# FifthEpoch/longcat-video-tta

Measured on AMD Instinct MI355X. Metric: denoised latent frames/sec (49x720p, 50-step CFG denoise), higher is better.
Workload: dtype bf16

## Files before the change

### longcat-video-tta_amd/csrc/attn_fwd_w64.hip

```cpp
#include "lcv_common.h"
#include <type_traits>

typedef __attribute__((address_space(3))) unsigned char lds_u8w;
#define AS3W __attribute__((address_space(3)))
#define SCHED_FENCE() __builtin_amdgcn_sched_barrier(0)

struct AttnFwdW64Params {
  const bf16_t* q;
  const bf16_t* k;
  const bf16_t* v;
  bf16_t* o;
  float* lse;
  int64_t Nq, Nk;
  int H;
  int64_t q_sb, q_sn, q_sh, k_sb, k_sn, k_sh, v_sb, v_sn, v_sh, o_sb, o_sn, o_sh;
  float scale;
  int gx, xcd_remap;
};

#define W64_RESCALE_THR 6.0f


__device__ __forceinline__ float w64_half_max(float v) {
  float a = v, b = v;
  asm volatile("s_nop 1\n\tv_permlane32_swap_b32 %0, %1\n\ts_nop 0" : "+v"(a), "+v"(b));
  return fmaxf(a, b);
}
__device__ __forceinline__ float w64_half_sum(float v) {
  float a = v, b = v;
  asm volatile("s_nop 1\n\tv_permlane32_swap_b32 %0, %1\n\ts_nop 0" : "+v"(a), "+v"(b));
  return a + b;
}
__device__ __forceinline__ float w_exp2(float x) { float y; asm volatile("v_exp_f32 %0, %1" : "=v"(y) : "v"(x)); return y; }
__device__ __forceinline__ float w_add(float a, float b) { float y; asm volatile("v_add_f32 %0, %1, %2" : "=v"(y) : "v"(a), "v"(b)); return y; }
__device__ __forceinline__ float w_max3(float a, float b, float c) { float y; asm volatile("v_max3_f32 %0, %1, %2, %3" : "=v"(y) : "v"(a), "v"(b), "v"(c)); return y; }
typedef __attribute__((ext_vector_type(2))) float f32x2w;
__device__ __forceinline__ f32x2w w_pk_add(f32x2w a, f32x2w b) { f32x2w y; asm volatile("v_pk_add_f32 %0, %1, %2" : "=v"(y) : "v"(a), "v"(b)); return y; }
__device__ __forceinline__ unsigned w_pack(float lo, float hi) { unsigned y; asm volatile("v_cvt_pk_bf16_f32 %0, %1, %2" : "=v"(y) : "v"(lo), "v"(hi)); return y; }

template <bool GUARD>
__device__ __forceinline__ void mfma_s(f32x16& c, const bf16x8& a, const bf16x8& b) {
  if constexpr (GUARD) asm volatile("s_nop 3\n\tv_mfma_f32_32x32x16_bf16 %0, %1, %2, %0" : "+v"(c) : "v"(a), "a"(b));
  else asm volatile("v_mfma_f32_32x32x16_bf16 %0, %1, %2, %0" : "+v"(c) : "v"(a), "a"(b));
}
template <bool GUARD>
__device__ __forceinline__ void mfma_s_first(f32x16& d, const f32x16& c, const bf16x8& a, const bf16x8& b) {
  if constexpr (GUARD) asm volatile("s_nop 3\n\tv_mfma_f32_32x32x16_bf16 %0, %2, %3, %1" : "=&v"(d) : "v"(c), "v"(a), "a"(b));
  else asm volatile("v_mfma_f32_32x32x16_bf16 %0, %2, %3, %1" : "=&v"(d) : "v"(c), "v"(a), "a"(b));
}
template <bool GUARD>
__device__ __forceinline__ void mfma_o(f32x16& c, const bf16x8& a, const bf16x8& b) {
  if constexpr (GUARD) asm volatile("s_nop 3\n\tv_mfma_f32_32x32x16_bf16 %0, %1, %2, %0" : "+a"(c) : "v"(a), "v"(b));
  else asm volatile("v_mfma_f32_32x32x16_bf16 %0, %1, %2, %0" : "+a"(c) : "v"(a), "v"(b));
}

#define SCW(S, nb, j) (S[(j) >> 4][nb][(j) & 15])

__global__ __launch_bounds__(256) void attn_fwd_w64_kernel(const AttnFwdW64Params p) {
  constexpr int TILE = 64 * 256;
  extern __shared__ __attribute__((aligned(16))) unsigned char smem[];
  lds_u8w* lds = (lds_u8w*)smem;
  constexpr int V_REGION = 2 * TILE;

  const int tid = threadIdx.x;
  const int lane = tid & 63;
  const int wave = __builtin_amdgcn_readfirstlane(tid >> 6);
  const int r = lane & 31, h = lane >> 5;
  int qb, head;
  int64_t b;
  if (p.xcd_remap) {
    const int id = blockIdx.x;
    const int xcd = id & 7, j = id >> 3;
    const int pair = (j / p.gx) * 8 + xcd;
    qb = j - (j / p.gx) * p.gx;
    head = pair % p.H;
    b = pair / p.H;
  } else {
    qb = blockIdx.x; head = blockIdx.y; b = blockIdx.z;
  }
  const int64_t q0 = (int64_t)qb * 256 + wave * 64;
  auto lane_now = []() -> int { return (int)__builtin_amdgcn_mbcnt_hi(~0u, __builtin_amdgcn_mbcnt_lo(~0u, 0u)); };
  const int nt = (int)((p.Nk + 63) / 64);
  const bool ragged = (p.Nk & 63) != 0;
  const char* kbase_u = lcv_uniform_ptr(p.k + b * p.k_sb + (int64_t)head * p.k_sh);
  const char* vbase_u = lcv_uniform_ptr(p.v + b * p.v_sb + (int64_t)head * p.v_sh);

  auto dma_row_of = [&](int ln, int i) { return 16 * wave + 4 * i + (ln >> 4); };
  auto dma_colb_of = [&](int ln, int i) {
    const int row = dma_row_of(ln, i);
    return 16 * ((ln & 15) ^ (((row & 3) << 2) | ((row >> 2) & 3)));
  };
  unsigned koff[4], voff[4];
#pragma unroll
  for (int i = 0; i < 4; ++i) {
    koff[i] = (unsigned)(dma_row_of(lane, i) * p.k_sn * 2 + dma_colb_of(lane, i));
    voff[i] = (unsigned)(dma_row_of(lane, i) * p.v_sn * 2 + dma_colb_of(lane, i));
  }
  auto last_off = [&](int i, int64_t sn) {
    const int ln = lane_now();
    int64_t row = (int64_t)(nt - 1) * 64 + dma_row_of(ln, i);
    if (row > p.Nk - 1) row = p.Nk - 1;
    return (unsigned)(row * sn * 2 + dma_colb_of(ln, i));
  };
  const unsigned lds_wave = (unsigned)(uintptr_t)lds + (unsigned)wave * 4096u;
  auto dma_one = [&](int which, int i, int dst_tile, int tile, bool known_full) __attribute__((always_inline)) {
    const int64_t sn = which ? p.v_sn : p.k_sn;
    const char* base = which ? vbase_u : kbase_u;
    unsigned off = which ? voff[i] : koff[i];
    if (!known_full && tile == nt - 1) off = last_off(i, sn);
    else base += (int64_t)tile * (128 * sn);
    asm volatile("s_mov_b32 m0, %2\n\ts_nop 0\n\tglobal_load_lds_dwordx4 %0, %1"
                 :: "v"(off), "s"(base), "s"(lds_wave + (unsigned)dst_tile + 1024u * i) : "memory", "m0");
  };
  auto dma_tile = [&](int which, int dst_tile, int tile) __attribute__((always_inline)) {
#pragma unroll
    for (int i = 0; i < 4; ++i) dma_one(which, i, dst_tile, tile, false);
  };
  constexpr int KOP = 0, VOP = 1;
  auto dma_wait_and_barrier = [&]() { asm volatile("s_waitcnt vmcnt(0)\n\ts_barrier" ::: "memory"); };

  int k_off[8];
  int v_off[2][4];
  auto set_read_offsets = [&](int ln, int slot) {
    const int rr = ln & 31, hh = ln >> 5;
    const int kfz = ((rr & 3) << 2) | ((rr >> 2) & 3);
#pragma unroll
    for (int ks = 0; ks < 8; ++ks) k_off[ks] = 256 * rr + 16 * ((2 * ks + hh) ^ kfz);
    const int q4 = (ln >> 2) & 3, p4 = ln & 3, g1 = (ln >> 4) & 1;
#pragma unroll
    for (int half = 0; half < 2; ++half)
#pragma unroll
      for (int d = 0; d < 4; ++d)
        v_off[half][d] = (int)(unsigned)(uintptr_t)lds + V_REGION + slot * TILE + 256 * (4 * hh + 8 * half + q4) + 8 * (p4 & 1) + 64 * (d ^ q4) +
                         16 * ((2 * g1 + (p4 >> 1)) ^ (hh + 2 * half));
  };
  set_read_offsets(lane, 2);
  auto read_k = [&](const lds_u8w* kb, int f) __attribute__((always_inline)) -> bf16x8 {
    return *reinterpret_cast<const AS3W bf16x8*>(kb + (f & 1) * 32 * 256 + k_off[f >> 1]);
  };
  auto read_v = [&](int g) __attribute__((always_inline)) -> bf16x8 {
    const s16x4 lo = __builtin_amdgcn_ds_read_tr16_b64_v4i16((AS3W s16x4*)(uintptr_t)(unsigned)(v_off[0][g & 3] + 4096 * (g >> 2)));
    const s16x4 hi = __builtin_amdgcn_ds_read_tr16_b64_v4i16((AS3W s16x4*)(uintptr_t)(unsigned)(v_off[1][g & 3] + 4096 * (g >> 2)));
    return __builtin_bit_cast(bf16x8, __builtin_shufflevector(lo, hi, 0, 1, 2, 3, 4, 5, 6, 7));
  };

  bf16x8 qf[2][8];
#pragma unroll
  for (int nb = 0; nb < 2; ++nb) {
    int64_t qrow = q0 + 32 * nb + r;
    if (qrow > p.Nq - 1) qrow = p.Nq - 1;
    const bf16_t* qp = p.q + b * p.q_sb + qrow * p.q_sn + (int64_t)head * p.q_sh + 8 * h;
#pragma unroll
    for (int ks = 0; ks < 8; ++ks) qf[nb][ks] = *reinterpret_cast<const bf16x8*>(qp + 16 * ks);
  }
#pragma unroll
  for (int nb = 0; nb < 2; ++nb)
#pragma unroll
    for (int ks = 0; ks < 8; ++ks) asm volatile("" : "+a"(qf[nb][ks]));

  f32x16 oacc[2][4];
#pragma unroll
  for (int nb = 0; nb < 2; ++nb)
#pragma unroll
    for (int d = 0; d < 4; ++d) {
#pragma unroll
      for (int e = 0; e < 16; ++e) oacc[nb][d][e] = 0.f;
      asm volatile("" : "+a"(oacc[nb][d]));
    }
  float m_run[2] = {0.f, 0.f}, l_run[2] = {0.f, 0.f};
  f32x16 minit[2];
#pragma unroll
  for (int nb = 0; nb < 2; ++nb)
#pragma unroll
    for (int e = 0; e < 16; ++e) minit[nb][e] = 0.f;
  f32x16 sa[2][2], sb[2][2];

  auto mask_last = [&](f32x16 (&s)[2][2]) __attribute__((always_inline)) {
    const int valid = (int)(p.Nk - (int64_t)(nt - 1) * 64);
    const int hh_ = lane_now() >> 5;
#pragma unroll
    for (int nb = 0; nb < 2; ++nb)
#pragma unroll
      for (int e = 0; e < 16; ++e) {
        const int key = (e & 3) + 8 * (e >> 2) + 4 * hh_;
        if (key >= valid) s[0][nb][e] = -INFINITY;
        if (key + 32 >= valid) s[1][nb][e] = -INFINITY;
      }
  };
  auto fence_o = [&]() __attribute__((always_inline)) {
    asm volatile("s_nop 15\n\ts_nop 15\n\ts_nop 15\n\ts_nop 15"
                 : "+a"(oacc[0][0]), "+a"(oacc[0][1]), "+a"(oacc[0][2]), "+a"(oacc[0][3]), "+a"(oacc[1][0]), "+a"(oacc[1][1]),
                   "+a"(oacc[1][2]), "+a"(oacc[1][3]));
  };
  auto fence_s = [&](f32x16 (&s)[2][2]) __attribute__((always_inline)) {
    asm volatile("s_nop 15\n\ts_nop 15\n\ts_nop 15\n\ts_nop 15" : "+v"(s[0][0]), "+v"(s[0][1]), "+v"(s[1][0]), "+v"(s[1][1]));
  };
  auto settle = [&](f32x16 (&s)[2][2], auto nb_c, float mx, bool first, bool need) __attribute__((always_inline)) {
    constexpr int nb = decltype(nb_c)::value;
    if (need || first) {
      fence_o();
      const float d = first ? mx : fmaxf(mx, 0.f);
      const float alpha = __builtin_amdgcn_exp2f(-d);
      m_run[nb] += d;
      l_run[nb] *= alpha;
#pragma unroll
      for (int dd = 0; dd < 4; ++dd)
#pragma unroll
        for (int e = 0; e < 16; ++e) oacc[nb][dd][e] *= alpha;
#pragma unroll
      for (int e = 0; e < 16; ++e) {
        s[0][nb][e] -= d;
        s[1][nb][e] -= d;
        asm volatile("v_mov_b32 %0, %1" : "+v"(minit[nb][e]) : "v"(-m_run[nb]));
      }
      fence_o();
    }
  };

#ifndef W64_PD
#define W64_PD 2
#endif
#ifndef W64_DMA_STRIDE
#define W64_DMA_STRIDE 1
#endif
  constexpr int PD = W64_PD, RING = PD + 1;
  bf16x8 kfr[RING], vfr[RING];
  int v_slot = 2;
  auto next_v_slot = [&]() __attribute__((always_inline)) -> int {
    v_slot = (v_slot == 2) ? 0 : v_slot + 1;
    return (v_slot == 0) ? -2 * TILE : TILE;
  };

  dma_tile(KOP, 0, 0);
  dma_tile(VOP, V_REGION, 0);
  dma_tile(KOP, TILE, 1);
  dma_tile(VOP, V_REGION + TILE, 1);
  dma_wait_and_barrier();
  {
#pragma unroll
    for (int kb_ = 0; kb_ < 2; ++kb_)
#pragma unroll
      for (int nb = 0; nb < 2; ++nb)
#pragma unroll
        for (int e = 0; e < 16; ++e) sa[kb_][nb][e] = 0.f;
#pragma unroll
    for (int f = 0; f < 16; ++f) {
      const bf16x8 a = read_k(lds, f);
      mfma_s<true>(sa[f & 1][0], a, qf[0][f >> 1]);
      mfma_s<true>(sa[f & 1][1], a, qf[1][f >> 1]);
    }
    fence_s(sa);
    auto first_settle = [&](auto nb_c) __attribute__((always_inline)) {
      constexpr int nb = decltype(nb_c)::value;
      float mx = sa[0][nb][0];
#pragma unroll
      for (int e = 1; e < 16; ++e) mx = fmaxf(mx, sa[0][nb][e]);
#pragma unroll
      for (int e = 0; e < 16; ++e) mx = fmaxf(mx, sa[1][nb][e]);
      settle(sa, nb_c, w64_half_max(mx), true, true);
    };
    first_settle(std::integral_constant<int, 0>{});
    first_settle(std::integral_constant<int, 1>{});
  }
  __syncthreads();
  dma_tile(KOP, 0, 2);
#pragma unroll
  for (int i = 0; i < PD; ++i) kfr[i] = read_k(lds + TILE, i);

  auto iteration = [&](const int t, auto par_c, auto steady_c, f32x16 (&c)[2][2], f32x16 (&n)[2][2]) __attribute__((always_inline)) {
    constexpr int PAR = decltype(par_c)::value;
    constexpr bool STEADY = decltype(steady_c)::value;
    const lds_u8w* kb = lds + (PAR ^ 1) * TILE;
    const lds_u8w* kb_next = lds + PAR * TILE;
    const bool has_k3 = STEADY || t + 3 < nt;
    const bool has_v2 = STEADY || t + 2 < nt;
    const int v_delta = next_v_slot();
    const int v_dst = V_REGION + ((v_slot == 0) ? 2 : v_slot - 1) * TILE;
    f32x2w psum[2];
    f32x2w ex[2][16];
    unsigned pw[2][16];
    SCHED_FENCE();
#pragma unroll
    for (int i = 0; i < 32; ++i) {
      const int f = i >> 1, nb = i & 1;
      if (nb == 0) {
        if (f + PD < 16) kfr[(f + PD) % RING] = read_k(kb, f + PD);
        if (f >= 16 - PD) vfr[f - (16 - PD)] = read_v(f - (16 - PD));
      }
      if (f < 2) {
        if (STEADY && i >= 1) mfma_s_first<false>(n[f & 1][nb], minit[nb], kfr[f % RING], qf[nb][0]);
        else mfma_s_first<true>(n[f & 1][nb], minit[nb], kfr[f % RING], qf[nb][0]);
      } else {
        if (STEADY) mfma_s<false>(n[f & 1][nb], kfr[f % RING], qf[nb][f >> 1]);
        else mfma_s<true>(n[f & 1][nb], kfr[f % RING], qf[nb][f >> 1]);
      }
      SCHED_FENCE();
      if (i >= 10 && i < 18) asm volatile("v_add_u32 %0, %1, %0" : "+v"(v_off[(i - 10) >> 2][(i - 10) & 3]) : "s"(v_delta));
      const int e_lo = (3 * i + 1) / 2, e_hi = (3 * (i + 1) + 1) / 2;
      const int a_lo = i ? (3 * (i - 1) + 1) / 2 : 0, a_hi = i ? e_lo : 0;
#pragma unroll
      for (int u = 0; u < 2; ++u) {
        const int x = e_lo + u;
        if (x < e_hi) ex[x & 1][x >> 2][(x >> 1) & 1] = w_exp2(SCW(c, x & 1, x >> 1));
      }
#pragma unroll
      for (int u = 0; u < 2; ++u) {
        const int x = a_lo + u;
        if (x < a_hi) {
          const int b_ = x & 1, j = x >> 1;
          if (j & 1) {
            pw[b_][j >> 1] = w_pack(ex[b_][j >> 1][0], ex[b_][j >> 1][1]);
            if (j == 3) psum[b_] = w_pk_add(ex[b_][0], ex[b_][1]);
            else if (j > 3) psum[b_] = w_pk_add(psum[b_], ex[b_][j >> 1]);
          }
        }
      }
      SCHED_FENCE();
    }
    if constexpr (!STEADY) {
      fence_s(n);
      if (t + 1 == nt - 1 && ragged) mask_last(n);
    }
    dma_wait_and_barrier();
    float mxa[2] = {0.f, 0.f}, mxb[2] = {0.f, 0.f}, mxh[2] = {0.f, 0.f};
    bool need[2] = {false, false};
    SCHED_FENCE();
#pragma unroll
    for (int j = 0; j < 32; ++j) {
      const int g = j >> 1, nb = j & 1;
      if (nb == 0) {
        if (g + PD < 16) vfr[(g + PD) % RING] = read_v(g + PD);
        if (g >= 16 - PD) kfr[g - (16 - PD)] = read_k(kb_next, g - (16 - PD));
      }
      const int kk = g >> 2;
      const u32x4 pbw = {pw[nb][4 * kk], pw[nb][4 * kk + 1], pw[nb][4 * kk + 2], pw[nb][4 * kk + 3]};
      if (STEADY && j >= 2) mfma_o<false>(oacc[nb][g & 3], vfr[g % RING], __builtin_bit_cast(bf16x8, pbw));
      else mfma_o<true>(oacc[nb][g & 3], vfr[g % RING], __builtin_bit_cast(bf16x8, pbw));
      SCHED_FENCE();
      if (j % W64_DMA_STRIDE == 0 && j / W64_DMA_STRIDE < 8) {
        const int dj = j / W64_DMA_STRIDE;
        if (dj < 4) { if (has_k3) dma_one(KOP, dj & 3, (PAR ^ 1) * TILE, t + 3, STEADY); }
        else { if (has_v2) dma_one(VOP, dj & 3, v_dst, t + 2, STEADY); }
      }
      if (j < 16) {
        const int b_ = j & 1, s_ = j >> 1;
        if (s_ == 0) {
          mxa[b_] = w_max3(n[0][b_][0], n[0][b_][1], n[0][b_][2]);
          mxb[b_] = w_max3(n[1][b_][0], n[1][b_][1], n[1][b_][2]);
        } else if (s_ < 7) {
          mxa[b_] = w_max3(mxa[b_], n[0][b_][2 * s_ + 1], n[0][b_][2 * s_ + 2]);
          mxb[b_] = w_max3(mxb[b_], n[1][b_][2 * s_ + 1], n[1][b_][2 * s_ + 2]);
        } else {
          mxa[b_] = w_max3(mxa[b_], n[0][b_][15], mxb[b_]);
          mxb[b_] = w_max3(mxa[b_], n[1][b_][15], n[1][b_][14]);
        }
      }
      if (j == 16 || j == 17) mxh[j & 1] = w64_half_max(mxb[j & 1]);
      if (j == 18 || j == 19) need[j & 1] = __builtin_amdgcn_ballot_w64(mxh[j & 1] > W64_RESCALE_THR) != 0ull;
      if (j == 0) {
        psum[1] = w_pk_add(psum[1], ex[1][11]);
        pw[1][11] = w_pack(ex[1][11][0], ex[1][11][1]);
      }
      if (j >= 6 && j < 22) {
        const int b_ = j & 1, el = 24 + ((j - 6) >> 1);
        ex[b_][el >> 1][el & 1] = w_exp2(SCW(c, b_, el));
      }
      if (j >= 8 && j < 24) {
        const int b_ = j & 1, el = 24 + ((j - 8) >> 1);
        if (el & 1) {
          psum[b_] = w_pk_add(psum[b_], ex[b_][el >> 1]);
          pw[b_][el >> 1] = w_pack(ex[b_][el >> 1][0], ex[b_][el >> 1][1]);
        }
      }
      if (j == 24 || j == 25) psum[j & 1][0] = w_add(psum[j & 1][0], psum[j & 1][1]);
      if (j == 26 || j == 27) l_run[j & 1] = w_add(l_run[j & 1], psum[j & 1][0]);
      SCHED_FENCE();
    }
    settle(n, std::integral_constant<int, 0>{}, mxh[0], false, need[0]);
    settle(n, std::integral_constant<int, 1>{}, mxh[1], false, need[1]);
  };

  auto final_tile = [&](f32x16 (&c)[2][2]) __attribute__((always_inline)) {
    const int v_delta = next_v_slot();
#pragma unroll
    for (int i = 0; i < 8; ++i) v_off[i >> 2][i & 3] += v_delta;
    unsigned pw[2][16];
#pragma unroll
    for (int nb = 0; nb < 2; ++nb) {
      float psum = 0.f;
      float ex[32];
#pragma unroll
      for (int j = 0; j < 32; ++j) {
        ex[j] = __builtin_amdgcn_exp2f(SCW(c, nb, j));
        psum += ex[j];
      }
      l_run[nb] += psum;
#pragma unroll
      for (int m = 0; m < 16; ++m) pw[nb][m] = w_pack(ex[2 * m], ex[2 * m + 1]);
    }
#pragma unroll
    for (int g = 0; g < 16; ++g) {
      const bf16x8 vf_ = read_v(g);
      const int kk = g >> 2;
#pragma unroll
      for (int nb = 0; nb < 2; ++nb) {
        const u32x4 pbw = {pw[nb][4 * kk], pw[nb][4 * kk + 1], pw[nb][4 * kk + 2], pw[nb][4 * kk + 3]};
        mfma_o<true>(oacc[nb][g & 3], vf_, __builtin_bit_cast(bf16x8, pbw));
      }
    }
    fence_o();
  };

  {
    using P0 = std::integral_constant<int, 0>;
    using P1 = std::integral_constant<int, 1>;
    int t = 0;
    for (; t + 5 < nt; t += 2) {
      iteration(t, P0{}, std::true_type{}, sa, sb);
      iteration(t + 1, P1{}, std::true_type{}, sb, sa);
    }
    fence_o(); fence_s(sa); fence_s(sb);
    for (; t + 1 <= nt - 2; t += 2) {
      iteration(t, P0{}, std::false_type{}, sa, sb);
      iteration(t + 1, P1{}, std::false_type{}, sb, sa);
    }
    if (t == nt - 2) iteration(t, P0{}, std::false_type{}, sa, sb);
    fence_o(); fence_s(sa); fence_s(sb);
    set_read_offsets(lane_now(), v_slot);
    if ((nt - 1) & 1) final_tile(sb);
    else final_tile(sa);
  }

  const int lane_l = lane_now();
  const int r_l = lane_l & 31, h_l = lane_l >> 5;
#pragma unroll
  for (int nb = 0; nb < 2; ++nb) {
    const float l_tot = w64_half_sum(l_run[nb]);
    const float inv = 1.0f / l_tot;
    const int64_t qrow = q0 + 32 * nb + r_l;
    if (qrow < p.Nq) {
      bf16_t* op = p.o + b * p.o_sb + qrow * p.o_sn + (int64_t)head * p.o_sh;
#pragma unroll
      for (int d = 0; d < 4; ++d)
#pragma unroll
        for (int i = 0; i < 4; ++i) {
          u16x4 pk;
#pragma unroll
          for (int e = 0; e < 4; ++e) pk[e] = f2bf(oacc[nb][d][4 * i + e] * inv);
          *reinterpret_cast<u16x4*>(op + 32 * d + 8 * i + 4 * h_l) = pk;
        }
      if (p.lse && h_l == 0) p.lse[(b * p.H + head) * p.Nq + qrow] = m_run[nb] * p.scale + __logf(l_tot);
    }
  }
}

int attn_fwd_w64_launch(const void* q, const void* k, const void* v, void* o, float* lse, int64_t B, int64_t H, int64_t Nq,
                        int64_t Nk, int64_t q_sb, int64_t q_sn, int64_t q_sh, int64_t k_sb, int64_t k_sn, int64_t k_sh,
                        int64_t v_sb, int64_t v_sn, int64_t v_sh, int64_t o_sb, int64_t o_sn, int64_t o_sh, float scale,
                        int xcd_ok, hipStream_t s) {
  AttnFwdW64Params p;
  p.q = (const bf16_t*)q; p.k = (const bf16_t*)k; p.v = (const bf16_t*)v; p.o = (bf16_t*)o; p.lse = lse;
  p.Nq = Nq; p.Nk = Nk; p.H = (int)H;
  p.q_sb = q_sb; p.q_sn = q_sn; p.q_sh = q_sh; p.k_sb = k_sb; p.k_sn = k_sn; p.k_sh = k_sh;
  p.v_sb = v_sb; p.v_sn = v_sn; p.v_sh = v_sh; p.o_sb = o_sb; p.o_sn = o_sn; p.o_sh = o_sh;
  p.scale = scale;
  const unsigned gx = (unsigned)((Nq + 255) / 256);
  p.gx = (int)gx;
  p.xcd_remap = (xcd_ok && (B * H) % 8 == 0 && gx >= 8) ? 1 : 0;
  const size_t lds = 5 * 64 * 256;
  static const bool attr_ok = !(hipFuncSetAttribute((const void*)attn_fwd_w64_kernel, hipFuncAttributeMaxDynamicSharedMemorySize, (int)lds) != hipSuccess);
  if (!attr_ok) {
      lcv_set_error("attn_fwd_w64: cannot raise dynamic LDS");
      return LCV_EDEVICE;
  }
  const dim3 grid = p.xcd_remap ? dim3(gx * (unsigned)(H * B)) : dim3(gx, (unsigned)H, (unsigned)B);
  hipLaunchKernelGGL(attn_fwd_w64_kernel, grid, dim3(256), lds, s, p);
  LCV_LAUNCH_CHECK("attn_fwd_w64");
  return LCV_OK;
}
```

Before: 0.06033.

## Schedule softmax VALU work into MFMA gaps via a compile-time checked op table

Replaces the formula-driven interleaving of exp, pack, sum, max and DMA issue between MFMAs with explicit constexpr per-gap tables, checked by static_asserts for completeness and a per-gap cycle budget. The row sum switches from packed v_pk_add_f32 to scalar adds, and the DMA issue is split so the m0 setup and the global_load_lds go in separate gaps. The aim is to fill each MFMA shadow more evenly and keep VALU work off the critical path. The cost is more scalar adds and a fixed hand-tuned schedule.

```diff
diff --git a/longcat-video-tta_amd/csrc/attn_fwd_w64.hip b/longcat-video-tta_amd/csrc/attn_fwd_w64.hip
--- a/longcat-video-tta_amd/csrc/attn_fwd_w64.hip
+++ b/longcat-video-tta_amd/csrc/attn_fwd_w64.hip
@@ -34,9 +34,118 @@
 __device__ __forceinline__ float w_exp2(float x) { float y; asm volatile("v_exp_f32 %0, %1" : "=v"(y) : "v"(x)); return y; }
 __device__ __forceinline__ float w_add(float a, float b) { float y; asm volatile("v_add_f32 %0, %1, %2" : "=v"(y) : "v"(a), "v"(b)); return y; }
 __device__ __forceinline__ float w_max3(float a, float b, float c) { float y; asm volatile("v_max3_f32 %0, %1, %2, %3" : "=v"(y) : "v"(a), "v"(b), "v"(c)); return y; }
-typedef __attribute__((ext_vector_type(2))) float f32x2w;
-__device__ __forceinline__ f32x2w w_pk_add(f32x2w a, f32x2w b) { f32x2w y; asm volatile("v_pk_add_f32 %0, %1, %2" : "=v"(y) : "v"(a), "v"(b)); return y; }
 __device__ __forceinline__ unsigned w_pack(float lo, float hi) { unsigned y; asm volatile("v_cvt_pk_bf16_f32 %0, %1, %2" : "=v"(y) : "v"(lo), "v"(hi)); return y; }
+
+template <int I, int N, class F>
+__device__ __forceinline__ void w64_static_for(F&& f) {
+  if constexpr (I < N) { f(std::integral_constant<int, I>{}); w64_static_for<I + 1, N>(f); }
+}
+enum : unsigned char { W64_NONE, W64_EXP, W64_ADD, W64_PACK, W64_LRUN, W64_VOFF, W64_MAX, W64_HMAX, W64_BALLOT, W64_M0, W64_DMA };
+struct W64Op { unsigned char kind, b, e; };
+constexpr int W64_SLOTS = 6;
+constexpr W64Op W64_P1[32][W64_SLOTS] = {
+  {{W64_EXP, 0, 0}, {W64_EXP, 1, 0}},
+  {{W64_EXP, 0, 1}},
+  {{W64_PACK, 0, 0}, {W64_ADD, 0, 1}, {W64_EXP, 1, 1}, {W64_EXP, 0, 2}},
+  {{W64_ADD, 0, 2}, {W64_PACK, 1, 0}, {W64_ADD, 1, 1}, {W64_EXP, 1, 2}},
+  {{W64_ADD, 1, 2}, {W64_EXP, 0, 3}, {W64_EXP, 1, 3}},
+  {{W64_PACK, 0, 1}, {W64_ADD, 0, 3}, {W64_PACK, 1, 1}, {W64_ADD, 1, 3}, {W64_EXP, 0, 4}},
+  {{W64_ADD, 0, 4}, {W64_EXP, 1, 4}, {W64_EXP, 0, 5}},
+  {{W64_PACK, 0, 2}, {W64_ADD, 0, 5}, {W64_ADD, 1, 4}, {W64_EXP, 1, 5}},
+  {{W64_PACK, 1, 2}, {W64_ADD, 1, 5}, {W64_EXP, 0, 6}, {W64_EXP, 1, 6}},
+  {{W64_ADD, 0, 6}, {W64_ADD, 1, 6}, {W64_EXP, 0, 7}},
+  {{W64_VOFF, 0, 0}, {W64_PACK, 0, 3}, {W64_ADD, 0, 7}, {W64_EXP, 1, 7}, {W64_EXP, 0, 8}},
+  {{W64_VOFF, 1, 0}, {W64_ADD, 0, 8}, {W64_PACK, 1, 3}, {W64_ADD, 1, 7}, {W64_EXP, 1, 8}},
+  {{W64_VOFF, 2, 0}, {W64_ADD, 1, 8}, {W64_EXP, 0, 9}, {W64_EXP, 1, 9}},
+  {{W64_VOFF, 3, 0}, {W64_PACK, 0, 4}, {W64_ADD, 0, 9}, {W64_PACK, 1, 4}, {W64_ADD, 1, 9}, {W64_EXP, 0, 10}},
+  {{W64_VOFF, 4, 0}, {W64_ADD, 0, 10}, {W64_EXP, 1, 10}, {W64_EXP, 0, 11}},
+  {{W64_VOFF, 5, 0}, {W64_PACK, 0, 5}, {W64_ADD, 0, 11}, {W64_ADD, 1, 10}, {W64_EXP, 1, 11}},
+  {{W64_VOFF, 6, 0}, {W64_PACK, 1, 5}, {W64_ADD, 1, 11}, {W64_EXP, 0, 12}, {W64_EXP, 1, 12}},
+  {{W64_VOFF, 7, 0}, {W64_ADD, 0, 12}, {W64_ADD, 1, 12}, {W64_EXP, 0, 13}},
+  {{W64_PACK, 0, 6}, {W64_ADD, 0, 13}, {W64_EXP, 1, 13}, {W64_EXP, 0, 14}},
+  {{W64_ADD, 0, 14}, {W64_PACK, 1, 6}, {W64_ADD, 1, 13}, {W64_EXP, 1, 14}},
+  {{W64_ADD, 1, 14}, {W64_EXP, 0, 15}, {W64_EXP, 1, 15}},
+  {{W64_PACK, 0, 7}, {W64_ADD, 0, 15}, {W64_PACK, 1, 7}, {W64_ADD, 1, 15}, {W64_EXP, 0, 16}},
+  {{W64_ADD, 0, 16}, {W64_EXP, 1, 16}, {W64_EXP, 0, 17}},
+  {{W64_PACK, 0, 8}, {W64_ADD, 0, 17}, {W64_ADD, 1, 16}, {W64_EXP, 1, 17}},
+  {{W64_PACK, 1, 8}, {W64_ADD, 1, 17}, {W64_EXP, 0, 18}, {W64_EXP, 1, 18}},
+  {{W64_ADD, 0, 18}, {W64_ADD, 1, 18}, {W64_EXP, 0, 19}},
+  {{W64_PACK, 0, 9}, {W64_ADD, 0, 19}, {W64_EXP, 1, 19}, {W64_EXP, 0, 20}},
+  {{W64_ADD, 0, 20}, {W64_PACK, 1, 9}, {W64_ADD, 1, 19}, {W64_EXP, 1, 20}},
+  {{W64_ADD, 1, 20}, {W64_EXP, 0, 21}, {W64_EXP, 1, 21}},
+  {{W64_PACK, 0, 10}, {W64_ADD, 0, 21}, {W64_PACK, 1, 10}, {W64_ADD, 1, 21}, {W64_EXP, 0, 22}},
+  {{W64_ADD, 0, 22}, {W64_EXP, 1, 22}, {W64_EXP, 0, 23}},
+  {{W64_PACK, 0, 11}, {W64_ADD, 0, 23}, {W64_ADD, 1, 22}, {W64_EXP, 1, 23}},
+};
+constexpr W64Op W64_P2[32][W64_SLOTS] = {
+  {{W64_M0, 0, 0}, {W64_PACK, 1, 11}, {W64_ADD, 1, 23}, {W64_EXP, 0, 24}, {W64_DMA, 0, 0}},
+  {{W64_ADD, 0, 24}, {W64_EXP, 1, 24}},
+  {{W64_M0, 1, 0}, {W64_ADD, 1, 24}, {W64_EXP, 0, 25}, {W64_DMA, 1, 0}},
+  {{W64_PACK, 0, 12}, {W64_ADD, 0, 25}},
+  {{W64_M0, 2, 0}, {W64_EXP, 1, 25}, {W64_DMA, 2, 0}},
+  {{W64_PACK, 1, 12}, {W64_ADD, 1, 25}, {W64_EXP, 0, 26}},
+  {{W64_M0, 3, 0}, {W64_ADD, 0, 26}, {W64_DMA, 3, 0}},
+  {{W64_EXP, 1, 26}},
+  {{W64_M0, 4, 0}, {W64_ADD, 1, 26}, {W64_MAX, 0, 0}, {W64_EXP, 0, 27}, {W64_DMA, 4, 0}},
+  {{W64_PACK, 0, 13}, {W64_ADD, 0, 27}, {W64_MAX, 1, 0}},
+  {{W64_M0, 5, 0}, {W64_MAX, 0, 1}, {W64_EXP, 1, 27}, {W64_DMA, 5, 0}},
+  {{W64_PACK, 1, 13}, {W64_ADD, 1, 27}, {W64_MAX, 1, 1}, {W64_EXP, 0, 28}},
+  {{W64_M0, 6, 0}, {W64_ADD, 0, 28}, {W64_MAX, 0, 2}, {W64_EXP, 1, 28}, {W64_DMA, 6, 0}},
+  {{W64_ADD, 1, 28}, {W64_MAX, 1, 2}},
+  {{W64_M0, 7, 0}, {W64_MAX, 0, 3}, {W64_EXP, 0, 29}, {W64_DMA, 7, 0}},
+  {{W64_PACK, 0, 14}, {W64_ADD, 0, 29}, {W64_MAX, 1, 3}, {W64_EXP, 1, 29}},
+  {{W64_PACK, 1, 14}, {W64_ADD, 1, 29}, {W64_MAX, 0, 4}},
+  {{W64_MAX, 1, 4}, {W64_EXP, 0, 30}},
+  {{W64_ADD, 0, 30}, {W64_MAX, 0, 5}, {W64_EXP, 1, 30}},
+  {{W64_ADD, 1, 30}, {W64_MAX, 1, 5}},
+  {{W64_MAX, 0, 6}, {W64_EXP, 0, 31}},
+  {{W64_PACK, 0, 15}, {W64_ADD, 0, 31}, {W64_MAX, 1, 6}, {W64_EXP, 1, 31}},
+  {{W64_PACK, 1, 15}, {W64_ADD, 1, 31}, {W64_LRUN, 0, 0}, {W64_MAX, 0, 7}},
+  {{W64_LRUN, 1, 0}, {W64_MAX, 1, 7}},
+  {{W64_HMAX, 0, 0}},
+  {{W64_HMAX, 1, 0}},
+  {{W64_BALLOT, 0, 0}},
+  {{W64_BALLOT, 1, 0}},
+  {},
+  {},
+  {},
+  {},
+};
+constexpr int w64_op_cost(W64Op o) {
+  return o.kind == W64_EXP ? 8 : o.kind == W64_PACK ? 5 : o.kind == W64_MAX ? 8 : o.kind == W64_HMAX ? 20 :
+         o.kind == W64_NONE ? 0 : 4;
+}
+constexpr int w64_read_cost(int phase, int i) {
+  return !(i & 1) || i > 29 ? 0 : ((phase == 1 && i >= 27) || (phase == 2 && i <= 25)) ? 12 : 8;
+}
+constexpr bool w64_table_ok(const W64Op (&t)[32][W64_SLOTS], int phase, int max_cyc, int max_exp) {
+  for (int i = 0; i < 32; ++i) {
+    int c = w64_read_cost(phase, i), ex = 0;
+    for (int s = 0; s < W64_SLOTS; ++s) { c += w64_op_cost(t[i][s]); ex += t[i][s].kind == W64_EXP; }
+    if (c > max_cyc || ex > max_exp) return false;
+  }
+  return true;
+}
+constexpr bool w64_table_complete() {
+  int exp_at[2][32] = {}, add_at[2][32] = {}, pack_at[2][16] = {}, n = 0;
+  for (int b = 0; b < 2; ++b) for (int e = 0; e < 32; ++e) { exp_at[b][e] = -1; add_at[b][e] = -1; }
+  for (int b = 0; b < 2; ++b) for (int m = 0; m < 16; ++m) pack_at[b][m] = -1;
+  for (int g = 0; g < 64; ++g)
+    for (int s = 0; s < W64_SLOTS; ++s) {
+      const W64Op o = g < 32 ? W64_P1[g][s] : W64_P2[g - 32][s];
+      const int at = 8 * g + s;
+      if (o.kind == W64_EXP) { if (exp_at[o.b][o.e] >= 0) return false; exp_at[o.b][o.e] = at; ++n; }
+      if (o.kind == W64_ADD) { if (o.e == 0 || exp_at[o.b][o.e] < 0 || (o.e > 1 && add_at[o.b][o.e - 1] < 0)) return false; add_at[o.b][o.e] = at; }
+      if (o.kind == W64_PACK) { if (exp_at[o.b][2 * o.e] < 0 || exp_at[o.b][2 * o.e + 1] < 0) return false; pack_at[o.b][o.e] = at; }
+      if (o.kind == W64_LRUN && add_at[o.b][31] < 0) return false;
+    }
+  for (int b = 0; b < 2; ++b)
+    for (int m = 0; m < 16; ++m)
+      if (pack_at[b][m] < 0 || pack_at[b][m] >= 8 * (32 + 8 * (m / 4) + b - 1) + W64_SLOTS) return false;
+  return n == 64;
+}
+static_assert(w64_table_complete(), "attn_fwd_w64 gap table: an exp, add or pack is missing, doubled or out of order");
+static_assert(w64_table_ok(W64_P1, 1, 38, 2) && w64_table_ok(W64_P2, 2, 37, 1), "attn_fwd_w64 gap table over its budget");
 
 template <bool GUARD>
 __device__ __forceinline__ void mfma_s(f32x16& c, const bf16x8& a, const bf16x8& b) {
@@ -112,6 +221,17 @@
     asm volatile("s_mov_b32 m0, %2\n\ts_nop 0\n\tglobal_load_lds_dwordx4 %0, %1"
                  :: "v"(off), "s"(base), "s"(lds_wave + (unsigned)dst_tile + 1024u * i) : "memory", "m0");
   };
+  auto dma_m0 = [&](int i, int dst_tile) __attribute__((always_inline)) {
+    asm volatile("s_mov_b32 m0, %0" :: "s"(lds_wave + (unsigned)dst_tile + 1024u * i) : "memory", "m0");
+  };
+  auto dma_req = [&](int which, int i, int tile, bool known_full) __attribute__((always_inline)) {
+    const int64_t sn = which ? p.v_sn : p.k_sn;
+    const char* base = which ? vbase_u : kbase_u;
+    unsigned off = which ? voff[i] : koff[i];
+    if (!known_full && tile == nt - 1) off = last_off(i, sn);
+    else base += (int64_t)tile * (128 * sn);
+    asm volatile("global_load_lds_dwordx4 %0, %1" :: "v"(off), "s"(base) : "memory");
+  };
   auto dma_tile = [&](int which, int dst_tile, int tile) __attribute__((always_inline)) {
 #pragma unroll
     for (int i = 0; i < 4; ++i) dma_one(which, i, dst_tile, tile, false);
@@ -219,9 +339,6 @@
 
 #ifndef W64_PD
 #define W64_PD 2
-#endif
-#ifndef W64_DMA_STRIDE
-#define W64_DMA_STRIDE 1
 #endif
   constexpr int PD = W64_PD, RING = PD + 1;
   bf16x8 kfr[RING], vfr[RING];
@@ -276,12 +393,46 @@
     const bool has_v2 = STEADY || t + 2 < nt;
     const int v_delta = next_v_slot();
     const int v_dst = V_REGION + ((v_slot == 0) ? 2 : v_slot - 1) * TILE;
-    f32x2w psum[2];
-    f32x2w ex[2][16];
+    float psum[2];
+    float ex[2][32];
     unsigned pw[2][16];
+    float mxa[2] = {0.f, 0.f}, mxb[2] = {0.f, 0.f}, mxh[2] = {0.f, 0.f};
+    bool need[2] = {false, false};
+    auto run_op = [&](auto phase_c, auto gap_c, auto slot_c) __attribute__((always_inline)) {
+      constexpr W64Op o = decltype(phase_c)::value == 1 ? W64_P1[decltype(gap_c)::value][decltype(slot_c)::value]
+                                                        : W64_P2[decltype(gap_c)::value][decltype(slot_c)::value];
+      constexpr int b_ = o.b, e = o.e;
+      if constexpr (o.kind == W64_EXP) ex[b_][e] = w_exp2(SCW(c, b_, e));
+      if constexpr (o.kind == W64_ADD) psum[b_] = w_add((e == 1) ? ex[b_][0] : psum[b_], ex[b_][e]);
+      if constexpr (o.kind == W64_PACK) pw[b_][e] = w_pack(ex[b_][2 * e], ex[b_][2 * e + 1]);
+      if constexpr (o.kind == W64_LRUN) l_run[b_] = w_add(l_run[b_], psum[b_]);
+      if constexpr (o.kind == W64_VOFF) asm volatile("v_add_u32 %0, %1, %0" : "+v"(v_off[b_ >> 2][b_ & 3]) : "s"(v_delta));
+      if constexpr (o.kind == W64_MAX) {
+        if constexpr (e == 0) {
+          mxa[b_] = w_max3(n[0][b_][0], n[0][b_][1], n[0][b_][2]);
+          mxb[b_] = w_max3(n[1][b_][0], n[1][b_][1], n[1][b_][2]);
+        } else if constexpr (e < 7) {
+          mxa[b_] = w_max3(mxa[b_], n[0][b_][2 * e + 1], n[0][b_][2 * e + 2]);
+          mxb[b_] = w_max3(mxb[b_], n[1][b_][2 * e + 1], n[1][b_][2 * e + 2]);
+        } else {
+          mxa[b_] = w_max3(mxa[b_], n[0][b_][15], mxb[b_]);
+          mxb[b_] = w_max3(mxa[b_], n[1][b_][15], n[1][b_][14]);
+        }
+      }
+      if constexpr (o.kind == W64_HMAX) mxh[b_] = w64_half_max(mxb[b_]);
+      if constexpr (o.kind == W64_BALLOT) need[b_] = __builtin_amdgcn_ballot_w64(mxh[b_] > W64_RESCALE_THR) != 0ull;
+      if constexpr (o.kind == W64_M0) {
+        if constexpr (b_ < 4) { if (has_k3) dma_m0(b_, (PAR ^ 1) * TILE); }
+        else { if (has_v2) dma_m0(b_ & 3, v_dst); }
+      }
+      if constexpr (o.kind == W64_DMA) {
+        if constexpr (b_ < 4) { if (has_k3) dma_req(KOP, b_, t + 3, STEADY); }
+        else { if (has_v2) dma_req(VOP, b_ & 3, t + 2, STEADY); }
+      }
+    };
     SCHED_FENCE();
-#pragma unroll
-    for (int i = 0; i < 32; ++i) {
+    w64_static_for<0, 32>([&](auto i_c) __attribute__((always_inline)) {
+      constexpr int i = decltype(i_c)::value;
       const int f = i >> 1, nb = i & 1;
       if (nb == 0) {
         if (f + PD < 16) kfr[(f + PD) % RING] = read_k(kb, f + PD);
@@ -295,38 +446,17 @@
         else mfma_s<true>(n[f & 1][nb], kfr[f % RING], qf[nb][f >> 1]);
       }
       SCHED_FENCE();
-      if (i >= 10 && i < 18) asm volatile("v_add_u32 %0, %1, %0" : "+v"(v_off[(i - 10) >> 2][(i - 10) & 3]) : "s"(v_delta));
-      const int e_lo = (3 * i + 1) / 2, e_hi = (3 * (i + 1) + 1) / 2;
-      const int a_lo = i ? (3 * (i - 1) + 1) / 2 : 0, a_hi = i ? e_lo : 0;
-#pragma unroll
-      for (int u = 0; u < 2; ++u) {
-        const int x = e_lo + u;
-        if (x < e_hi) ex[x & 1][x >> 2][(x >> 1) & 1] = w_exp2(SCW(c, x & 1, x >> 1));
-      }
-#pragma unroll
-      for (int u = 0; u < 2; ++u) {
-        const int x = a_lo + u;
-        if (x < a_hi) {
-          const int b_ = x & 1, j = x >> 1;
-          if (j & 1) {
-            pw[b_][j >> 1] = w_pack(ex[b_][j >> 1][0], ex[b_][j >> 1][1]);
-            if (j == 3) psum[b_] = w_pk_add(ex[b_][0], ex[b_][1]);
-            else if (j > 3) psum[b_] = w_pk_add(psum[b_], ex[b_][j >> 1]);
-          }
-        }
-      }
+      w64_static_for<0, W64_SLOTS>([&](auto s_c) { run_op(std::integral_constant<int, 1>{}, i_c, s_c); });
       SCHED_FENCE();
-    }
+    });
     if constexpr (!STEADY) {
       fence_s(n);
       if (t + 1 == nt - 1 && ragged) mask_last(n);
     }
     dma_wait_and_barrier();
-    float mxa[2] = {0.f, 0.f}, mxb[2] = {0.f, 0.f}, mxh[2] = {0.f, 0.f};
-    bool need[2] = {false, false};
     SCHED_FENCE();
-#pragma unroll
-    for (int j = 0; j < 32; ++j) {
+    w64_static_for<0, 32>([&](auto j_c) __attribute__((always_inline)) {
+      constexpr int j = decltype(j_c)::value;
       const int g = j >> 1, nb = j & 1;
       if (nb == 0) {
         if (g + PD < 16) vfr[(g + PD) % RING] = read_v(g + PD);
@@ -337,45 +467,9 @@
       if (STEADY && j >= 2) mfma_o<false>(oacc[nb][g & 3], vfr[g % RING], __builtin_bit_cast(bf16x8, pbw));
       else mfma_o<true>(oacc[nb][g & 3], vfr[g % RING], __builtin_bit_cast(bf16x8, pbw));
       SCHED_FENCE();
-      if (j % W64_DMA_STRIDE == 0 && j / W64_DMA_STRIDE < 8) {
-        const int dj = j / W64_DMA_STRIDE;
-        if (dj < 4) { if (has_k3) dma_one(KOP, dj & 3, (PAR ^ 1) * TILE, t + 3, STEADY); }
-        else { if (has_v2) dma_one(VOP, dj & 3, v_dst, t + 2, STEADY); }
-      }
-      if (j < 16) {
-        const int b_ = j & 1, s_ = j >> 1;
-        if (s_ == 0) {
-          mxa[b_] = w_max3(n[0][b_][0], n[0][b_][1], n[0][b_][2]);
-          mxb[b_] = w_max3(n[1][b_][0], n[1][b_][1], n[1][b_][2]);
-        } else if (s_ < 7) {
-          mxa[b_] = w_max3(mxa[b_], n[0][b_][2 * s_ + 1], n[0][b_][2 * s_ + 2]);
-          mxb[b_] = w_max3(mxb[b_], n[1][b_][2 * s_ + 1], n[1][b_][2 * s_ + 2]);
-        } else {
-          mxa[b_] = w_max3(mxa[b_], n[0][b_][15], mxb[b_]);
-          mxb[b_] = w_max3(mxa[b_], n[1][b_][15], n[1][b_][14]);
-        }
-      }
-      if (j == 16 || j == 17) mxh[j & 1] = w64_half_max(mxb[j & 1]);
-      if (j == 18 || j == 19) need[j & 1] = __builtin_amdgcn_ballot_w64(mxh[j & 1] > W64_RESCALE_THR) != 0ull;
-      if (j == 0) {
-        psum[1] = w_pk_add(psum[1], ex[1][11]);
-        pw[1][11] = w_pack(ex[1][11][0], ex[1][11][1]);
-      }
-      if (j >= 6 && j < 22) {
-        const int b_ = j & 1, el = 24 + ((j - 6) >> 1);
-        ex[b_][el >> 1][el & 1] = w_exp2(SCW(c, b_, el));
-      }
-      if (j >= 8 && j < 24) {
-        const int b_ = j & 1, el = 24 + ((j - 8) >> 1);
-        if (el & 1) {
-          psum[b_] = w_pk_add(psum[b_], ex[b_][el >> 1]);
-          pw[b_][el >> 1] = w_pack(ex[b_][el >> 1][0], ex[b_][el >> 1][1]);
-        }
-      }
-      if (j == 24 || j == 25) psum[j & 1][0] = w_add(psum[j & 1][0], psum[j & 1][1]);
-      if (j == 26 || j == 27) l_run[j & 1] = w_add(l_run[j & 1], psum[j & 1][0]);
+      w64_static_for<0, W64_SLOTS>([&](auto s_c) { run_op(std::integral_constant<int, 2>{}, j_c, s_c); });
       SCHED_FENCE();
-    }
+    });
     settle(n, std::integral_constant<int, 0>{}, mxh[0], false, need[0]);
     settle(n, std::integral_constant<int, 1>{}, mxh[1], false, need[1]);
   };
```

Result: faster. 0.06293, median of 6 (+4.3%).
